# SkyworkAI/Vitron

Measured on NVIDIA H100. Metric: Vicuna-7B generated tokens/s, batch-8 x (256 vision + 512 text) prefill + 128-token greedy decode, incl. ViT-L/14 encode, higher is better.
Workload: dtype bf16

## Files before the change

### include/vitron_b200.h

```cpp
#ifndef VITRON_B200_H_
#define VITRON_B200_H_

#include <stddef.h>
#include <stdint.h>

#ifdef __cplusplus
extern "C" {
#endif

#ifndef __CUDA_RUNTIME_H__
typedef struct CUstream_st* cudaStream_t;
#endif

#define VB_ACT_NONE 0
#define VB_ACT_GELU 1
#define VB_ACT_QUICK_GELU 2
#define VB_ACT_RELU 3
#define VB_ACT_SILU 4

#define VB_GLU_NONE 0
#define VB_GLU_SWIGLU 1
#define VB_GLU_GEGLU 2

typedef struct vb_epilogue {
  const void* bias;
  const void* rowbias;
  int64_t rowbias_rows;
  const void* residual;
  int64_t ldr;
  float alpha;
  int32_t act;
  int32_t glu;
  int32_t out_fp32;
  const float* rowscale;
  float rms_eps;
} vb_epilogue;

const char* vb200_version(void);
const char* vb200_last_error(void);
int vb200_device_ok(void);
int vb200_set_pdl(int enable);
int vb200_set_attention_impl(int impl);
int vb200_attention_watchdog(uint32_t* out3);
int vb200_attention_tc_occupancy(int head_dim);

size_t vb200_gemm_bf16_workspace_size(int64_t M, int64_t N, int64_t K);
int vb200_gemm_bf16(const void* A, int64_t lda, const void* W, int64_t ldw, void* out, int64_t ldo,
                    int64_t M, int64_t N, int64_t K, const vb_epilogue* epi, void* workspace,
                    size_t workspace_bytes, cudaStream_t stream);

int vb200_gemm_nf4(const void* A, int64_t lda, const void* codes, const void* scales, const float* kscale, void* out,
                   int64_t ldo, int64_t M, int64_t N, int64_t K, const vb_epilogue* epi, cudaStream_t stream);
int vb200_nf4_dequant(const void* codes, const void* scales, const float* kscale, void* out, int64_t N, int64_t K,
                      cudaStream_t stream);



size_t vb200_conv_nhwc_workspace_size(int64_t nb, int64_t h, int64_t w, int64_t cin, int64_t cout, int kh, int kw,
                                      int stride, int pad_h, int pad_w);
int vb200_conv_nhwc_bf16(const void* X, const void* Wt, void* out, int64_t nb, int64_t h,
                         int64_t w, int64_t cin, int64_t cout, int kh, int kw, int stride,
                         int pad_h, int pad_w, const vb_epilogue* epi, void* workspace,
                         size_t workspace_bytes, cudaStream_t stream);
int vb200_set_gemm_impl(int impl);
int vb200_set_gemm_debug(int resident_b, int dbg);

int vb200_conv_nhwc_direct(const void* X, const void* Wt, const void* bias, void* out, int64_t nb,
                           int64_t h, int64_t w, int64_t cin, int64_t cout, int kh, int kw,
                           int stride, int pad_h, int pad_w, cudaStream_t stream);

int vb200_rmsnorm(const void* x, int64_t ldx, const void* weight, void* out, int64_t ldo,
                  int64_t rows, int64_t d, float eps, cudaStream_t stream);
int vb200_row_rstd(const void* x, int64_t ldx, float* out, int64_t rows, int64_t d, float eps,
                   cudaStream_t stream);
int vb200_layernorm(const void* x, int64_t ldx, const void* weight, const void* bias, void* out,
                    int64_t ldo, int64_t rows, int64_t d, float eps, cudaStream_t stream);
size_t vb200_groupnorm_workspace_size(int64_t n, int64_t groups, int64_t c);
int vb200_groupnorm_nhwc(const void* x, const void* weight, const void* bias, void* out, int64_t n,
                         int64_t spatial, int64_t c, int64_t groups, float eps, int act,
                         void* workspace, size_t workspace_bytes, cudaStream_t stream);

int vb200_attention(const void* q, const void* k, const void* v, void* out, int64_t B, int64_t H,
                    int64_t Sq, int64_t Skv, int64_t head_dim, int64_t q_sb, int64_t q_ss,
                    int64_t q_sh, int64_t k_sb, int64_t k_ss, int64_t k_sh, int64_t v_sb,
                    int64_t v_ss, int64_t v_sh, int64_t o_sb, int64_t o_ss, int64_t o_sh,
                    float scale, int causal, const int32_t* kv_len, const uint8_t* mask,
                    int64_t m_sb, int64_t m_sh, int64_t m_sq, cudaStream_t stream);
size_t vb200_attention_workspace_size(int64_t B, int64_t H, int64_t Sq, int64_t Skv, int64_t head_dim, int causal);
int vb200_attention_ws(const void* q, const void* k, const void* v, void* out, int64_t B, int64_t H,
                       int64_t Sq, int64_t Skv, int64_t head_dim, int64_t q_sb, int64_t q_ss,
                       int64_t q_sh, int64_t k_sb, int64_t k_ss, int64_t k_sh, int64_t v_sb,
                       int64_t v_ss, int64_t v_sh, int64_t o_sb, int64_t o_ss, int64_t o_sh,
                       float scale, int causal, const int32_t* kv_len, const uint8_t* mask,
                       int64_t m_sb, int64_t m_sh, int64_t m_sq, void* workspace, size_t workspace_bytes,
                       cudaStream_t stream);
size_t vb200_attention_paged_workspace_size(int64_t B, int64_t H, int64_t Sq, int64_t head_dim, int64_t max_kv_len);
int vb200_attention_paged(const void* q, int64_t q_sb, int64_t q_ss, int64_t q_sh, const void* k_pages,
                          const void* v_pages, int64_t num_pages, const int32_t* block_table, int64_t max_pages,
                          const int32_t* q_start, const int32_t* q_len, void* out, int64_t o_sb, int64_t o_ss,
                          int64_t o_sh, int64_t B, int64_t H, int64_t Sq, int64_t head_dim, int64_t page_size,
                          int64_t max_kv_len, float scale, void* workspace, size_t workspace_bytes,
                          cudaStream_t stream);
int vb200_attention_short(const void* q, const void* k, const void* v, void* out, int64_t nseq,
                          int64_t H, int64_t S, int64_t head_dim, int64_t q_sb, int64_t q_ss,
                          int64_t q_sh, int64_t k_sb, int64_t k_ss, int64_t k_sh, int64_t v_sb,
                          int64_t v_ss, int64_t v_sh, int64_t o_sb, int64_t o_ss, int64_t o_sh,
                          int64_t inner, int64_t q_so, int64_t k_so, int64_t v_so, int64_t o_so,
                          float scale, cudaStream_t stream);

int vb200_rope_kv_append(void* qkv, int64_t ld_qkv, const int32_t* positions,
                         const int32_t* batch_of_token, const int32_t* slot_of_token, void* k_pages,
                         void* v_pages, const int32_t* block_table, int64_t max_pages,
                         int64_t tokens, int64_t n_heads, int64_t head_dim, int64_t page_size,
                         float rope_theta, cudaStream_t stream);
size_t vb200_attn_decode_workspace_size(int64_t B, int64_t n_heads, int64_t head_dim,
                                        int64_t max_splits);
int vb200_attn_decode_paged(const void* q, int64_t ld_q, const void* k_pages, const void* v_pages,
                            const int32_t* block_table, int64_t max_pages, const int32_t* kv_len,
                            void* out, int64_t ld_o, int64_t B, int64_t n_heads, int64_t head_dim,
                            int64_t page_size, int64_t max_kv_len, float scale, void* workspace,
                            size_t workspace_bytes, cudaStream_t stream);
int vb200_rope_table(const int32_t* positions, float* table, int64_t B, int64_t head_dim, float rope_theta,
                     cudaStream_t stream);
int vb200_attn_decode_rope(const void* qkv, int64_t ld_qkv, const float* rope_table, void* k_pages,
                           void* v_pages, const int32_t* block_table, int64_t max_pages,
                           const int32_t* kv_len, void* out, int64_t ld_o, int64_t B, int64_t n_heads,
                           int64_t head_dim, int64_t page_size, int64_t max_kv_len, float scale,
                           void* workspace, size_t workspace_bytes, cudaStream_t stream);
int vb200_attn_decode_rope_beam(const void* qkv, int64_t ld_qkv, const float* rope_table, void* k_pages,
                                void* v_pages, const int32_t* block_table, int64_t max_pages, const int32_t* kv_len,
                                const int32_t* beam_src, int64_t src_ld, const int32_t* gen_start, void* out,
                                int64_t ld_o, int64_t B, int64_t n_heads, int64_t head_dim, int64_t page_size,
// ... 101 lines not shown
```

### vitron_b200/_lib.py

```python
import ctypes as C
import os

_HERE = os.path.dirname(os.path.abspath(__file__))
LIB_PATH = os.path.join(_HERE, "libvitron_b200.so")

ACT_NONE, ACT_GELU, ACT_QUICK_GELU, ACT_RELU, ACT_SILU = 0, 1, 2, 3, 4
GLU_NONE, GLU_SWIGLU, GLU_GEGLU = 0, 1, 2

_ERR = {-1: "VB_ERR_ARG", -2: "VB_ERR_CUDA", -3: "VB_ERR_WORKSPACE", -4: "VB_ERR_UNSUPPORTED",
        -5: "VB_ERR_DRIVER"}


class Epilogue(C.Structure):
    _fields_ = [
        ("bias", C.c_void_p), ("rowbias", C.c_void_p), ("rowbias_rows", C.c_int64),
        ("residual", C.c_void_p), ("ldr", C.c_int64), ("alpha", C.c_float),
        ("act", C.c_int32), ("glu", C.c_int32), ("out_fp32", C.c_int32),
        ("rowscale", C.c_void_p), ("rms_eps", C.c_float),
    ]


_p, _i64, _i32, _f, _sz = C.c_void_p, C.c_int64, C.c_int, C.c_float, C.c_size_t

SIGNATURES = {
    "vb200_version": (C.c_char_p, []),
    "vb200_last_error": (C.c_char_p, []),
    "vb200_device_ok": (_i32, []),
    "vb200_set_pdl": (_i32, [_i32]),
    "vb200_set_attention_impl": (_i32, [_i32]),
    "vb200_attention_watchdog": (_i32, [_p]),
    "vb200_attention_tc_occupancy": (_i32, [_i32]),
    "vb200_gemm_bf16_workspace_size": (_sz, [_i64, _i64, _i64]),
    "vb200_gemm_bf16": (_i32, [_p, _i64, _p, _i64, _p, _i64, _i64, _i64, _i64, C.POINTER(Epilogue), _p, _sz, _p]),
    "vb200_gemm_nf4": (_i32, [_p, _i64, _p, _p, _p, _p, _i64, _i64, _i64, _i64, C.POINTER(Epilogue), _p]),
    "vb200_nf4_dequant": (_i32, [_p, _p, _p, _p, _i64, _i64, _p]),
    "vb200_conv_nhwc_workspace_size": (_sz, [_i64, _i64, _i64, _i64, _i64, _i32, _i32, _i32, _i32, _i32]),
    "vb200_conv_nhwc_bf16": (_i32, [_p, _p, _p, _i64, _i64, _i64, _i64, _i64, _i32, _i32, _i32, _i32, _i32,
                                    C.POINTER(Epilogue), _p, _sz, _p]),
    "vb200_set_gemm_impl": (_i32, [_i32]),
    "vb200_set_gemm_debug": (_i32, [_i32, _i32]),
    "vb200_conv_nhwc_direct": (_i32, [_p, _p, _p, _p, _i64, _i64, _i64, _i64, _i64, _i32, _i32, _i32, _i32, _i32, _p]),
    "vb200_rmsnorm": (_i32, [_p, _i64, _p, _p, _i64, _i64, _i64, _f, _p]),
    "vb200_row_rstd": (_i32, [_p, _i64, _p, _i64, _i64, _f, _p]),
    "vb200_layernorm": (_i32, [_p, _i64, _p, _p, _p, _i64, _i64, _i64, _f, _p]),
    "vb200_groupnorm_workspace_size": (_sz, [_i64, _i64, _i64]),
    "vb200_groupnorm_nhwc": (_i32, [_p, _p, _p, _p, _i64, _i64, _i64, _i64, _f, _i32, _p, _sz, _p]),
    "vb200_attention": (_i32, [_p, _p, _p, _p, _i64, _i64, _i64, _i64, _i64] + [_i64] * 12 +
                        [_f, _i32, _p, _p, _i64, _i64, _i64, _p]),
    "vb200_attention_workspace_size": (_sz, [_i64, _i64, _i64, _i64, _i64, _i32]),
    "vb200_attention_ws": (_i32, [_p, _p, _p, _p, _i64, _i64, _i64, _i64, _i64] + [_i64] * 12 +
                           [_f, _i32, _p, _p, _i64, _i64, _i64, _p, _sz, _p]),
    "vb200_attention_paged_workspace_size": (_sz, [_i64, _i64, _i64, _i64, _i64]),
    "vb200_attention_paged": (_i32, [_p, _i64, _i64, _i64, _p, _p, _i64, _p, _i64, _p, _p, _p, _i64, _i64, _i64,
                                     _i64, _i64, _i64, _i64, _i64, _i64, _f, _p, _sz, _p]),
    "vb200_attention_short": (_i32, [_p, _p, _p, _p, _i64, _i64, _i64, _i64] + [_i64] * 17 + [_f, _p]),
    "vb200_add_rowgroup": (_i32, [_p, _p, _p, _i64, _i64, _i64, _i64, _p]),
    "vb200_rope_kv_append": (_i32, [_p, _i64, _p, _p, _p, _p, _p, _p, _i64, _i64, _i64, _i64, _i64, _f, _p]),
    "vb200_attn_decode_workspace_size": (_sz, [_i64, _i64, _i64, _i64]),
    "vb200_attn_decode_paged": (_i32, [_p, _i64, _p, _p, _p, _i64, _p, _p, _i64, _i64, _i64, _i64, _i64, _i64,
                                       _f, _p, _sz, _p]),
    "vb200_rope_table": (_i32, [_p, _p, _i64, _i64, _f, _p]),
    "vb200_attn_decode_rope": (_i32, [_p, _i64, _p, _p, _p, _p, _i64, _p, _p, _i64, _i64, _i64, _i64, _i64, _i64,
                                      _f, _p, _sz, _p]),
    "vb200_attn_decode_rope_beam": (_i32, [_p, _i64, _p, _p, _p, _p, _i64, _p, _p, _i64, _p, _p, _i64, _i64, _i64, _i64,
                                           _i64, _i64, _f, _p, _sz, _p]),
    "vb200_splice_multimodal": (_i32, [_p, _i64, _p, _i64, _p, _p, _i64, _i64, _p]),
    "vb200_argmax_rows": (_i32, [_p, _i32, _i64, _i64, _i64, _p, _p]),
    "vb200_argmax_advance": (_i32, [_p, _i64, _i64, _i64, _p, _p, _p, _p, _p, _i64, _p, _p]),
    "vb200_sample_advance": (_i32, [_p, _i64, _i64, _i64, _p, _p, _p, _p, _p, _p, _i64, _p, _p]),
    "vb200_beam_workspace_size": (_sz, [_i64]),
    "vb200_beam_advance": (_i32, [_p, _i64, _i64, _i64, _i64, _p, _p, _p, _p, _p, _i64, _p, _p, _p, _p, _p, _i64, _p, _p,
                                  _p, _p, _i64, _p, _p, _sz, _p]),
    "vb200_beam_sample_advance": (_i32, [_p, _i64, _i64, _i64, _i64, _p, _p, _p, _p, _p, _i64, _p, _p, _p, _p, _p, _i64,
                                         _p, _p, _p, _p, _i64, _p, _p, _sz, _p, _p]),
    "vb200_patchify": (_i32, [_p, _i32, _p, _i64, _i64, _i64, _i64, _i64, _i64, _p]),
    "vb200_vit_embed_ln": (_i32, [_p, _p, _p, _p, _p, _p, _i64, _i64, _i64, _f, _p]),
    "vb200_upsample2x_nhwc": (_i32, [_p, _p, _i64, _i64, _i64, _i64, _p]),
    "vb200_add_bf16": (_i32, [_p, _p, _p, _i64, _i64, _p]),
    "vb200_cfg_combine": (_i32, [_p, _p, _p, _f, _i64, _p]),
    "vb200_region_mask_pool": (_i32, [_p, _p, _p, _i64, _i64, _i64, _i64, _p]),
    "vb200_seem_attn_mask": (_i32, [_p, _p, _i64, _i64, _i64, _i64, _i64, _p]),
    "vb200_resize_bilinear_nhwc": (_i32, [_p, _p, _i64, _i64, _i64, _i64, _i64, _i64, _p]),
    "vb200_softmax_rows": (_i32, [_p, _i64, _p, _i64, _i64, _i64, _p]),
    "vb200_preprocess_frames": (_i32, [_p, _p] + [_i64] * 11 + [_p, _p, _i32, _i32, _i32, _p]),
    "vb200_im2col_nchw": (_i32, [_p, _i32, _p] + [_i64] * 10 + [_p]),
    "vb200_set_dwconv_impl": (_i32, [_i32]),
    "vb200_dwconv_nhwc": (_i32, [_p, _i64, _p, _p, _i64, _i64, _i64, _i64, _i64, _i32, _p]),
    "vb200_colmean_workspace_size": (_sz, [_i64, _i64, _i64]),
    "vb200_colmean": (_i32, [_p, _p, _i64, _i64, _i64, _i32, _p, _sz, _p]),
    "vb200_focal_modulate": (_i32, [_p, _i64, _p, _i64, _p, _p, _i64, _i64, _i64, _f, _p]),
    "vb200_mul_rows": (_i32, [_p, _i64, _p, _i64, _p, _i64, _i64, _p]),
    "vb200_layernorm_add": (_i32, [_p, _i64, _p, _p, _p, _i64, _p, _i64, _i64, _i64, _f, _p]),
}

_lib = None


def load():
    global _lib
    if _lib is not None:
        return _lib
    if not os.path.exists(LIB_PATH):
        raise RuntimeError(
            f"{LIB_PATH} is missing: build it with `python -m vitron_b200.build` "
            "(nvcc, sm_90a). vitron_b200 has no CPU fallback.")
    lib = C.CDLL(LIB_PATH)
    for name, (res, args) in SIGNATURES.items():
        fn = getattr(lib, name)
        fn.restype = res
        fn.argtypes = args
    _lib = lib
    mode = os.environ.get("VB200_GEMM_MODE")
    if mode:
# ... 13 lines not shown
```

### vitron_b200/csrc/gemm.cu

```cuda
#include <cstdlib>
#include "gemm_v2.cuh"

namespace vb {

__global__ void splitk_reduce_kernel(const float* __restrict__ ws, int splits,
                                     long long split_stride, long long ws_ld, int rows, int ncols,
                                     void* out, long long ldo, const bf16* __restrict__ bias,
                                     const bf16* __restrict__ rowbias, int rowbias_rows,
                                     const bf16* __restrict__ residual, long long ldr, float alpha,
                                     int act, int glu, int out_fp32, const float* __restrict__ rowscale) {
  pdl_trigger();
  pdl_wait();
  const int n_out_total = glu != VB_GLU_NONE ? ncols / 2 : ncols;
  const int groups = (n_out_total + 7) / 8;
  long long idx = blockIdx.x * static_cast<long long>(blockDim.x) + threadIdx.x;
  if (idx >= static_cast<long long>(rows) * groups) return;
  reduce_item(ws, splits, split_stride, ws_ld, static_cast<int>(idx / groups), static_cast<int>(idx % groups) * 8,
              ncols, out, ldo, bias, rowbias, rowbias_rows, residual, ldr, alpha, act, glu, out_fp32, rowscale);
}

typedef CUresult (*PFN_encodeTiled)(CUtensorMap*, CUtensorMapDataType, cuuint32_t, void*,
                                    const cuuint64_t*, const cuuint64_t*, const cuuint32_t*,
                                    const cuuint32_t*, CUtensorMapInterleave, CUtensorMapSwizzle,
                                    CUtensorMapL2promotion, CUtensorMapFloatOOBfill);

static PFN_encodeTiled get_encode_fn() {
  static PFN_encodeTiled fn = nullptr;
  if (fn) return fn;
  void* p = nullptr;
  cudaDriverEntryPointQueryResult q;
  if (cudaGetDriverEntryPoint("cuTensorMapEncodeTiled", &p, cudaEnableDefault, &q) != cudaSuccess ||
      q != cudaDriverEntryPointSuccess)
    return nullptr;
  fn = reinterpret_cast<PFN_encodeTiled>(p);
  return fn;
}

static int make_tmap(CUtensorMap* m, const void* ptr, int rank, const uint64_t* dims,
                     const uint64_t* strides_bytes , const uint32_t* box,
                     const uint32_t* estr, CUtensorMapSwizzle swz = CU_TENSOR_MAP_SWIZZLE_128B) {
  PFN_encodeTiled fn = get_encode_fn();
  if (!fn) return VB_ERR_DRIVER;
  CUresult r = fn(m, CU_TENSOR_MAP_DATA_TYPE_BFLOAT16, rank, const_cast<void*>(ptr), dims,
                  strides_bytes, box, estr, CU_TENSOR_MAP_INTERLEAVE_NONE, swz,
                  CU_TENSOR_MAP_L2_PROMOTION_L2_256B, CU_TENSOR_MAP_FLOAT_OOB_FILL_NONE);
  return r == CUDA_SUCCESS ? VB_OK : VB_ERR_DRIVER;
}


static int swap_splits(long long M, long long N, long long K) {
  const int sms = vb_num_sms();
  const int m_blocks = static_cast<int>((N + BLOCK_M - 1) / BLOCK_M);
  const int kblocks = static_cast<int>((K + BLOCK_K - 1) / BLOCK_K);
  int best = 1;
  float best_score = -1.f;
  for (int s = 1; s <= 32 && s <= kblocks; ++s) {
    if (static_cast<size_t>(s) * M * N * sizeof(float) > (static_cast<size_t>(96) << 20)) break;
    const long long units = static_cast<long long>(m_blocks) * s;
    const long long waves = (units + sms - 1) / sms;
    const float util = static_cast<float>(units) / static_cast<float>(waves * sms);
    const int per = (kblocks + s - 1) / s;
    const float bal = static_cast<float>(kblocks) / static_cast<float>(s * per);
    const float score = util * bal - 0.01f * static_cast<float>(s);
    if (score > best_score + 1e-6f) { best_score = score; best = s; }
  }
  return best;
}

static int validate_epi(const vb_epilogue* e, long long N) {
  if (e->glu != VB_GLU_NONE && (N % 32) != 0) return VB_ERR_ARG;
  if (e->act < VB_ACT_NONE || e->act > VB_ACT_SILU) return VB_ERR_ARG;
  if (e->glu < VB_GLU_NONE || e->glu > VB_GLU_GEGLU) return VB_ERR_ARG;
  return VB_OK;
}

static int g_gemm_impl = 0;
static int g_gemm_resb = 1;
static int g_gemm_dbg = 0;
int resb_smem_bytes(int bn, int nkb);

static int resb_tile(long long M, long long N, int nkb, int need) {
  if (g_gemm_impl == 1 || !(g_gemm_resb & 3) || (need != 0 && need != F_RES && need != F_GLU && need != F_ACT)) return 0;
  if (nkb > 5 && !(g_gemm_resb & 2)) return 0;
  if (M < 4096) return 0;
  const int cands[3] = {160, 256, 128};
  int best = 0;
  float best_cost = 1e30f;
  for (int i = 0; i < 3; ++i) {
    const int bn = cands[i];
    if (resb_smem_bytes(bn, nkb) > SMEM_LIMIT) continue;
    const long long nb = (N + bn - 1) / bn;
    if (nb > vb_num_sms()) continue;
    const int groups = vb_num_sms() / static_cast<int>(nb);
    const long long mb = (M + BLOCK_M - 1) / BLOCK_M;
    const long long per_cta = (mb + groups - 1) / groups;
    const float mma = static_cast<float>(bn) / 256.f, astream = bn == 160 ? 0.55f : 0.9f;
    const float cost = static_cast<float>(per_cta) * nkb * (mma > astream ? mma : astream);
    if (cost < best_cost) { best_cost = cost; best = bn; }
  }
  return best;
}

struct TilePlan {
  int bn, splits;
};

static TilePlan plan_tiles(long long mb, long long N, int kblocks, bool allow_split, long long out_rows) {
  const int sms = vb_num_sms();
  const int cands[5] = {256, 160, 128, 64, 32};
  const float tk[5] = {1.0f, 0.78f, 0.76f, 0.625f, 0.57f};
  TilePlan best = {256, 1};
  float best_t = 1e30f;
  if (const char* force = getenv("VB200_FORCE_BN")) {
    const int v = atoi(force);
    if (v == 256 || v == 160 || v == 128 || v == 64 || v == 32) return {v, 1};
  }
  for (int i = 0; i < 5; ++i) {
    const int bn = cands[i];
    const long long nbk = (N + bn - 1) / bn;
    const long long tiles = mb * nbk;
    for (int sp = 1; sp <= 8; ++sp) {
// ... 285 lines not shown
```

### vitron_b200/csrc/gemv.cu

```cuda
#include "common.cuh"
#include "vitron_b200.h"
#include <type_traits>

namespace vb {

struct GemvParams {
  const bf16* W; long long ldw;
  const bf16* X; long long ldx;
  void* out; long long ldo;
  int M, N, K;
  const bf16* bias; const bf16* rowbias; int rowbias_rows;
  const bf16* residual; long long ldr;
  float alpha; int act, glu, out_fp32;
  const float* rowscale; float rms_eps;
};

__device__ __forceinline__ float gemv_act(float x, int act) {
  switch (act) {
    case VB_ACT_GELU: return gelu_erf(x);
    case VB_ACT_QUICK_GELU: return quick_gelu(x);
    case VB_ACT_RELU: return fmaxf(x, 0.f);
    case VB_ACT_SILU: return silu(x);
    default: return x;
  }
}

__device__ __forceinline__ void mma16816(float (&c)[4], uint32_t a0, uint32_t a1, uint32_t a2, uint32_t a3,
                                         uint32_t b0, uint32_t b1) {
  asm("mma.sync.aligned.m16n8k16.row.col.f32.bf16.bf16.f32 {%0,%1,%2,%3}, {%4,%5,%6,%7}, {%8,%9}, {%0,%1,%2,%3};"
      : "+f"(c[0]), "+f"(c[1]), "+f"(c[2]), "+f"(c[3])
      : "r"(a0), "r"(a1), "r"(a2), "r"(a3), "r"(b0), "r"(b1));
}

__device__ __forceinline__ uint4 ldg_stream(const bf16* p, bool ok) {
  uint4 v = make_uint4(0, 0, 0, 0);
  if (ok) asm volatile("ld.global.nc.L1::no_allocate.v4.u32 {%0,%1,%2,%3}, [%4];" : "=r"(v.x), "=r"(v.y), "=r"(v.z), "=r"(v.w) : "l"(p));
  return v;
}
__device__ __forceinline__ uint4 ldg_cached(const bf16* p, bool ok) {
  uint4 v = make_uint4(0, 0, 0, 0);
  if (ok) v = __ldg(reinterpret_cast<const uint4*>(p));
  return v;
}

template <int ROWS, int NT>
__global__ void __launch_bounds__(256, 2) gemv_bf16_kernel(const GemvParams p) {
  constexpr int WARPS = 8;
  constexpr int RG = ROWS / 16;
  constexpr int KS = WARPS / RG;
  constexpr int G = 2;
  __shared__ float red[2][WARPS][16][NT * 8 + 1];
  __shared__ float red_sq[WARPS][NT * 8];
  __shared__ float rstd_s[NT * 8];

  const int warp = threadIdx.x >> 5, lane = threadIdx.x & 31;
  const int g = lane >> 2, t = lane & 3;
  const int rg = warp % RG, ks = warp / RG;
  const int ntiles = (p.N + ROWS - 1) / ROWS;
  const bf16* x0 = p.X + static_cast<long long>(min(g, p.M - 1)) * p.ldx;
  const bf16* x1 = p.X + static_cast<long long>(min(g + 8, p.M - 1)) * p.ldx;
  const bool x0ok = g < p.M, x1ok = (NT == 2) && (g + 8 < p.M);

  const int chunks = (p.K + 63) / 64;
  const int base = chunks / KS, rem = chunks % KS;
  const int c0 = ks * base + min(ks, rem);
  const int c1 = c0 + base + (ks < rem ? 1 : 0);
  const int ngroups = (c1 - c0 + G - 1) / G;
  const int npairs = (ngroups + 1) / 2;

  const bool do_rms = p.rms_eps > 0.f && p.rowscale == nullptr;
  float sq0 = 0.f, sq1 = 0.f;

  struct Buf { uint4 wl[G][2], wh[G][2]; };
  auto load_group = [&](Buf& bf, int tile, int grp) {
    const int row0 = tile * ROWS + rg * 16;
    const bf16* wa = p.W + static_cast<long long>(min(row0 + g, p.N - 1)) * p.ldw;
    const bf16* wb = p.W + static_cast<long long>(min(row0 + g + 8, p.N - 1)) * p.ldw;
    const bool live = tile < ntiles;
#pragma unroll
    for (int u = 0; u < G; ++u) {
      const int c = c0 + grp * G + u;
      const int k0 = c * 64 + 8 * t, k1 = k0 + 32;
      const bool in = live && c < c1;
      const bool ok0 = in && k0 < p.K, ok1 = in && k1 < p.K;
      bf.wl[u][0] = ldg_stream(wa + k0, ok0); bf.wl[u][1] = ldg_stream(wa + k1, ok1);
      bf.wh[u][0] = ldg_stream(wb + k0, ok0); bf.wh[u][1] = ldg_stream(wb + k1, ok1);
    }
  };
  float acc[NT][4];
  auto compute_group = [&](const Buf& bf, int grp, bool first_tile) {
    uint4 xa[G][2], xb[G][2];
#pragma unroll
    for (int u = 0; u < G; ++u) {
      const int c = c0 + grp * G + u;
      const int k0 = c * 64 + 8 * t, k1 = k0 + 32;
      const bool in = c < c1;
      const bool ok0 = in && k0 < p.K, ok1 = in && k1 < p.K;
      xa[u][0] = ldg_cached(x0 + k0, ok0 && x0ok); xa[u][1] = ldg_cached(x0 + k1, ok1 && x0ok);
      if (NT == 2) { xb[u][0] = ldg_cached(x1 + k0, ok0 && x1ok); xb[u][1] = ldg_cached(x1 + k1, ok1 && x1ok); }
    }
#pragma unroll
    for (int u = 0; u < G; ++u) {
      const uint32_t al[8] = {bf.wl[u][0].x, bf.wl[u][0].y, bf.wl[u][0].z, bf.wl[u][0].w, bf.wl[u][1].x, bf.wl[u][1].y, bf.wl[u][1].z, bf.wl[u][1].w};
      const uint32_t ah[8] = {bf.wh[u][0].x, bf.wh[u][0].y, bf.wh[u][0].z, bf.wh[u][0].w, bf.wh[u][1].x, bf.wh[u][1].y, bf.wh[u][1].z, bf.wh[u][1].w};
      const uint32_t b0[8] = {xa[u][0].x, xa[u][0].y, xa[u][0].z, xa[u][0].w, xa[u][1].x, xa[u][1].y, xa[u][1].z, xa[u][1].w};
      uint32_t b1[8] = {0, 0, 0, 0, 0, 0, 0, 0};
      if (NT == 2) {
        b1[0] = xb[u][0].x; b1[1] = xb[u][0].y; b1[2] = xb[u][0].z; b1[3] = xb[u][0].w;
        b1[4] = xb[u][1].x; b1[5] = xb[u][1].y; b1[6] = xb[u][1].z; b1[7] = xb[u][1].w;
      }
      if (do_rms && first_tile && rg == 0) {
#pragma unroll
        for (int j = 0; j < 8; ++j) {
          float2 f = unpack_bf16(b0[j]);
          sq0 += f.x * f.x + f.y * f.y;
          if (NT == 2) { float2 h2 = unpack_bf16(b1[j]); sq1 += h2.x * h2.x + h2.y * h2.y; }
        }
      }
#pragma unroll
      for (int j = 0; j < 4; ++j) {
        mma16816(acc[0], al[2 * j], ah[2 * j], al[2 * j + 1], ah[2 * j + 1], b0[2 * j], b0[2 * j + 1]);
        if (NT == 2) mma16816(acc[1], al[2 * j], ah[2 * j], al[2 * j + 1], ah[2 * j + 1], b1[2 * j], b1[2 * j + 1]);
      }
    }
  };

  Buf buf0, buf1;
  pdl_trigger();
  load_group(buf0, blockIdx.x, 0);
  load_group(buf1, blockIdx.x, 1);
  pdl_wait();

  const bool glu = p.glu != VB_GLU_NONE;
  const int out_cols = glu ? ROWS / 2 : ROWS;
  const int n_out_total = glu ? p.N / 2 : p.N;
  int par = 0;
  bool first = true;
  for (int tile = blockIdx.x; tile < ntiles; tile += gridDim.x) {
#pragma unroll
    for (int i = 0; i < NT; ++i) acc[i][0] = acc[i][1] = acc[i][2] = acc[i][3] = 0.f;
    for (int pr = 0; pr < npairs; ++pr) {
      const bool last = pr + 1 == npairs;
      compute_group(buf0, 2 * pr, first);
      if (!last) load_group(buf0, tile, 2 * pr + 2); else load_group(buf0, tile + gridDim.x, 0);
      compute_group(buf1, 2 * pr + 1, first);
      if (!last) load_group(buf1, tile, 2 * pr + 3); else load_group(buf1, tile + gridDim.x, 1);
    }
#pragma unroll
    for (int i = 0; i < NT; ++i) {
      red[par][warp][g][i * 8 + 2 * t] = acc[i][0];
      red[par][warp][g][i * 8 + 2 * t + 1] = acc[i][1];
      red[par][warp][g + 8][i * 8 + 2 * t] = acc[i][2];
      red[par][warp][g + 8][i * 8 + 2 * t + 1] = acc[i][3];
    }
    if (do_rms && first) {
      sq0 += __shfl_xor_sync(0xffffffffu, sq0, 1); sq0 += __shfl_xor_sync(0xffffffffu, sq0, 2);
      if (NT == 2) { sq1 += __shfl_xor_sync(0xffffffffu, sq1, 1); sq1 += __shfl_xor_sync(0xffffffffu, sq1, 2); }
      if (t == 0) { red_sq[warp][g] = sq0; if (NT == 2) red_sq[warp][8 + g] = sq1; }
    }
    __syncthreads();
    if (do_rms && first) {
      if (threadIdx.x < NT * 8) {
        float ss = 0.f;
#pragma unroll
        for (int s2 = 0; s2 < KS; ++s2) ss += red_sq[s2 * RG][threadIdx.x];
        rstd_s[threadIdx.x] = rsqrtf(ss / p.K + p.rms_eps);
      }
      __syncthreads();
    }
    for (int item = threadIdx.x; item < p.M * out_cols; item += 256) {
      const int tok = item / out_cols, j = item % out_cols;
      const int fa = j, fb = j + 16;
      const int na = tile * ROWS + fa;
      const int oc = glu ? tile * (ROWS / 2) + j : na;
      if (oc >= n_out_total) continue;
      float va = 0.f, vb_ = 0.f;
#pragma unroll
      for (int s2 = 0; s2 < KS; ++s2) {
        va += red[par][s2 * RG + fa / 16][fa % 16][tok];
        if (glu) vb_ += red[par][s2 * RG + (fb / 16) % RG][fb % 16][tok];
      }
      if (do_rms) { const float rs = rstd_s[tok]; va *= rs; vb_ *= rs; }
      else if (p.rowscale) { const float rs = p.rowscale[tok]; va *= rs; vb_ *= rs; }
      if (p.bias) {
        va += __bfloat162float(p.bias[na]);
        if (glu) vb_ += __bfloat162float(p.bias[na + 16]);
      }
      if (p.rowbias) {
        const bf16* rbp = p.rowbias + (tok / p.rowbias_rows) * static_cast<long long>(p.N);
        va += __bfloat162float(rbp[na]);
        if (glu) vb_ += __bfloat162float(rbp[na + 16]);
      }
      float r;
      if (p.glu == VB_GLU_SWIGLU) r = silu(va) * vb_;
      else if (p.glu == VB_GLU_GEGLU) r = va * gelu_erf(vb_);
      else r = gemv_act(va, p.act);
      if (p.residual) r = __bfloat162float(p.residual[tok * p.ldr + oc]) + p.alpha * r;
      else r *= p.alpha;
      if (p.out_fp32) reinterpret_cast<float*>(p.out)[tok * p.ldo + oc] = r;
      else reinterpret_cast<bf16*>(p.out)[tok * p.ldo + oc] = __float2bfloat16(r);
    }
    par ^= 1;
    first = false;
  }
}

}

using namespace vb;

int vb_launch_gemv(const void* A, int64_t lda, const void* W, int64_t ldw, void* out, int64_t ldo, int64_t M,
                   int64_t N, int64_t K, const vb_epilogue* e, cudaStream_t stream) {
  GemvParams p;
  p.W = reinterpret_cast<const bf16*>(W); p.ldw = ldw;
  p.X = reinterpret_cast<const bf16*>(A); p.ldx = lda;
  p.out = out; p.ldo = ldo;
  p.M = static_cast<int>(M); p.N = static_cast<int>(N); p.K = static_cast<int>(K);
  p.bias = reinterpret_cast<const bf16*>(e->bias);
  p.rowbias = reinterpret_cast<const bf16*>(e->rowbias);
  p.rowbias_rows = e->rowbias_rows > 0 ? static_cast<int>(e->rowbias_rows) : 1;
  p.residual = reinterpret_cast<const bf16*>(e->residual); p.ldr = e->ldr;
  p.alpha = e->alpha; p.act = e->act; p.glu = e->glu; p.out_fp32 = e->out_fp32;
  p.rowscale = e->rowscale; p.rms_eps = e->rms_eps;
  const bool glu = e->glu != VB_GLU_NONE;
  const bool rows32 = glu || (N / 16 > 6LL * vb_num_sms());
  const unsigned tiles = static_cast<unsigned>((N + (rows32 ? 31 : 15)) / (rows32 ? 32 : 16));
  const unsigned cap = 2u * static_cast<unsigned>(vb_num_sms());
  const unsigned grid = tiles < cap ? tiles : cap;
  cudaError_t err;
  if (M <= 8) {
    if (rows32) err = vb_launch(gemv_bf16_kernel<32, 1>, dim3(grid), dim3(256), 0, stream, p);
    else err = vb_launch(gemv_bf16_kernel<16, 1>, dim3(grid), dim3(256), 0, stream, p);
  } else {
    if (rows32) err = vb_launch(gemv_bf16_kernel<32, 2>, dim3(grid), dim3(256), 0, stream, p);
    else err = vb_launch(gemv_bf16_kernel<16, 2>, dim3(grid), dim3(256), 0, stream, p);
  }
  if (err != cudaSuccess) { vb_set_last_error(err); return VB_ERR_CUDA; }
  return VB_OK;
}
```

### vitron_b200/ops.py

```python
import ctypes as C
import math
import struct

import torch

from . import _lib, beam
from .nf4 import NF4Weight
from ._lib import (ACT_GELU, ACT_NONE, ACT_QUICK_GELU, ACT_RELU, ACT_SILU, GLU_GEGLU, GLU_NONE,
                   GLU_SWIGLU, Epilogue, check)

BF16 = torch.bfloat16
_ws = {}
_launches = [0]


def launch_count():
    return _launches[0]


def count_launches(n):
    _launches[0] += int(n)


def _stream():
# ... 259 lines not shown
    check(lib.vb200_layernorm(x2.data_ptr(), ldx, weight.data_ptr(), _ptr(bias), o2.data_ptr(), ldo, x2.shape[0],
                              x2.shape[1], float(eps), _stream()), "vb200_layernorm")
    _launches[0] += 1
    return out


def groupnorm_nhwc(x, weight, bias, groups, eps, act=ACT_NONE, n=None, out=None):
    lib = _lib.load()
    _req(x.is_contiguous() and x.dtype == BF16, "x must be contiguous bf16")
    c = x.shape[-1]
    n = x.shape[0] if n is None else n
    spatial = x.numel() // (n * c)
    out = torch.empty_like(x) if out is None else out
    need = lib.vb200_groupnorm_workspace_size(n, groups, c)
    ws = workspace(need, x.device, "gn")
    check(lib.vb200_groupnorm_nhwc(x.data_ptr(), weight.data_ptr(), bias.data_ptr(), out.data_ptr(), n, spatial, c,
                                   groups, float(eps), int(act), ws.data_ptr(), need, _stream()),
          "vb200_groupnorm_nhwc")
    _launches[0] += 1
    return out


def _bsh(t):
    _req(t.dim() == 4 and t.stride(3) == 1, "expect [B, S, H, D] with contiguous D")
    return t.stride(0), t.stride(1), t.stride(2)


def attention(q, k, v, scale=None, causal=False, kv_len=None, mask=None, out=None):
    lib = _lib.load()
    B, Sq, H, D = q.shape
    Skv = k.shape[1]
    scale = 1.0 / math.sqrt(D) if scale is None else scale
    if out is None:
        out = torch.empty((B, Sq, H, D), dtype=BF16, device=q.device)
    m_ptr, m_sb, m_sh, m_sq = 0, 0, 0, 0
    if mask is not None:
        if mask.dtype == torch.bool:
            mask = mask.view(torch.uint8)
        _req(mask.dim() == 4 and mask.stride(3) == 1 and mask.shape[2] == Sq and mask.shape[3] == Skv, "bad mask")
        m_ptr = mask.data_ptr()
        m_sb = mask.stride(0) if mask.shape[0] > 1 else 0
        m_sh = mask.stride(1) if mask.shape[1] > 1 else 0
        m_sq = mask.stride(2)
    need = lib.vb200_attention_workspace_size(B, H, Sq, Skv, D, 1 if causal else 0) if kv_len is None else 0
    ws = workspace(need, q.device, "attn") if need else None
    check(lib.vb200_attention_ws(q.data_ptr(), k.data_ptr(), v.data_ptr(), out.data_ptr(), B, H, Sq, Skv, D,
                                 *_bsh(q), *_bsh(k), *_bsh(v), *_bsh(out), float(scale), 1 if causal else 0,
                                 _ptr(kv_len), m_ptr, m_sb, m_sh, m_sq, _ptr(ws), need, _stream()), "vb200_attention_ws")
    _launches[0] += 2 if need else 1
    return out


def attention_paged(q, k_pages, v_pages, block_table, q_start, q_len, max_kv_len, scale=None, out=None):
    lib = _lib.load()
    B, Sq, H, D = q.shape
    scale = 1.0 / math.sqrt(D) if scale is None else scale
    _req(block_table.dim() == 2 and block_table.shape[0] >= B and block_table.is_contiguous(),
         "block_table: contiguous int32 [>= B, max_pages]")
    _req(k_pages.is_contiguous() and v_pages.is_contiguous() and k_pages.shape == v_pages.shape, "contiguous pages")
    if out is None:
        out = torch.empty((B, Sq, H, D), dtype=BF16, device=q.device)
    need = lib.vb200_attention_paged_workspace_size(B, H, Sq, D, int(max_kv_len))
    ws = workspace(need, q.device, "attn") if need else None
    check(lib.vb200_attention_paged(q.data_ptr(), *_bsh(q), k_pages.data_ptr(), v_pages.data_ptr(), k_pages.shape[0],
                                    block_table.data_ptr(), block_table.shape[1], q_start.data_ptr(), q_len.data_ptr(),
                                    out.data_ptr(), *_bsh(out), B, H, Sq, D, k_pages.shape[2], int(max_kv_len),
                                    float(scale), _ptr(ws), need, _stream()), "vb200_attention_paged")
    _launches[0] += 2 if need else 1
    return out


def set_attention_impl(impl):
    check(_lib.load().vb200_set_attention_impl(int(impl)), "vb200_set_attention_impl")


def attention_watchdog():
    import ctypes
    buf = (ctypes.c_uint32 * 3)()
    torch.cuda.synchronize()
    check(_lib.load().vb200_attention_watchdog(ctypes.addressof(buf)), "vb200_attention_watchdog")
    return tuple(buf)


def attention_short(q, k, v, scale=None, out=None):
    lib = _lib.load()
    scale = 1.0 / math.sqrt(q.shape[-1]) if scale is None else scale
    if out is None:
        out = torch.empty(q.shape, dtype=BF16, device=q.device)
    if q.dim() == 4:
        nseq, S, H, D = q.shape
        inner, so = 0, (0, 0, 0, 0)
        b3 = [_bsh(t) for t in (q, k, v, out)]
    else:
        _req(q.dim() == 5, "expect 4-D or 5-D q")
        outer, inner, S, H, D = q.shape
        nseq = outer * inner
        so = tuple(t.stride(0) for t in (q, k, v, out))
        for t in (q, k, v, out):
            _req(t.stride(4) == 1, "contiguous head dim")
        b3 = [(t.stride(1), t.stride(2), t.stride(3)) for t in (q, k, v, out)]
    check(lib.vb200_attention_short(q.data_ptr(), k.data_ptr(), v.data_ptr(), out.data_ptr(), nseq, H, S, D,
                                    *b3[0], *b3[1], *b3[2], *b3[3], inner, *so, float(scale), _stream()),
          "vb200_attention_short")
    _launches[0] += 1
    return out


def add_rowgroup(x, table, group_rows, period, out=None):
    lib = _lib.load()
    x2, _ = _rows2d(x)
    _req(x.is_contiguous() and table.is_contiguous(), "contiguous")
    out = torch.empty_like(x) if out is None else out
    check(lib.vb200_add_rowgroup(x2.data_ptr(), table.data_ptr(), out.data_ptr(), x2.shape[0], x2.shape[1],
                                 group_rows, period, _stream()), "vb200_add_rowgroup")
    _launches[0] += 1
    return out


def rope_kv_append(qkv, positions, n_heads, head_dim, theta, k_pages=None, v_pages=None, block_table=None,
                   batch_of_token=None, slot_of_token=None, page_size=0):
    lib = _lib.load()
    q2, ld = _rows2d(qkv)
    max_pages = block_table.shape[1] if block_table is not None else 0
    check(lib.vb200_rope_kv_append(q2.data_ptr(), ld, positions.data_ptr(), _ptr(batch_of_token),
                                   _ptr(slot_of_token), _ptr(k_pages), _ptr(v_pages), _ptr(block_table),
                                   max_pages, q2.shape[0], n_heads, head_dim, page_size, float(theta), _stream()),
          "vb200_rope_kv_append")
    _launches[0] += 1
    return qkv


def attn_decode_paged(q, k_pages, v_pages, block_table, kv_len, n_heads, head_dim, page_size, max_kv_len,
                      scale=None, out=None):
    lib = _lib.load()
    B = q.shape[0]
    scale = 1.0 / math.sqrt(head_dim) if scale is None else scale
    if out is None:
        out = torch.empty((B, n_heads * head_dim), dtype=BF16, device=q.device)
    need = lib.vb200_attn_decode_workspace_size(B, n_heads, head_dim, 32)
    ws = workspace(need, q.device, "dec")
    check(lib.vb200_attn_decode_paged(q.data_ptr(), q.stride(0), k_pages.data_ptr(), v_pages.data_ptr(),
                                      block_table.data_ptr(), block_table.shape[1], kv_len.data_ptr(),
                                      out.data_ptr(), out.stride(0), B, n_heads, head_dim, page_size, max_kv_len,
                                      float(scale), ws.data_ptr(), need, _stream()), "vb200_attn_decode_paged")
    _launches[0] += 1
    return out


def rope_table(positions, head_dim, theta, out=None):
    lib = _lib.load()
    B = positions.shape[0]
    if out is None:
        out = torch.empty((B, head_dim), dtype=torch.float32, device=positions.device)
    check(lib.vb200_rope_table(positions.data_ptr(), out.data_ptr(), B, head_dim, float(theta), _stream()),
          "vb200_rope_table")
    _launches[0] += 1
    return out


def attn_decode_rope(qkv, table, k_pages, v_pages, block_table, kv_len, n_heads, head_dim, page_size, max_kv_len,
                     scale=None, out=None):
    lib = _lib.load()
    B = qkv.shape[0]
    scale = 1.0 / math.sqrt(head_dim) if scale is None else scale
    if out is None:
        out = torch.empty((B, n_heads * head_dim), dtype=BF16, device=qkv.device)
# ... 361 lines not shown
```

Before: 1030.

## Stream GEMV weights through per-warp TMA mbarrier ring instead of register double-buffering

Replaces the register-level double-buffered streaming loads of weight tiles in the decode GEMV kernel with a per-warp 4-stage TMA ring in swizzled shared memory, synchronised by mbarriers. Weight prefetch for the first stages is issued before the PDL wait so it overlaps the previous kernel. The aim is deeper memory-level parallelism with fewer registers spent on in-flight loads. It adds about 66KB of dynamic shared memory per block, which may limit occupancy to fewer blocks per SM, a tensor-map encode on every launch, and a watchdog trap path plus occupancy query helpers.

```diff
diff --git a/include/vitron_b200.h b/include/vitron_b200.h
--- a/include/vitron_b200.h
+++ b/include/vitron_b200.h
@@ -48,6 +48,8 @@
 int vb200_gemm_bf16(const void* A, int64_t lda, const void* W, int64_t ldw, void* out, int64_t ldo,
                     int64_t M, int64_t N, int64_t K, const vb_epilogue* epi, void* workspace,
                     size_t workspace_bytes, cudaStream_t stream);
+int vb200_gemv_watchdog(uint32_t* out3);
+int vb200_gemv_occupancy(int32_t m, int32_t rows32);
 
 int vb200_gemm_nf4(const void* A, int64_t lda, const void* codes, const void* scales, const float* kscale, void* out,
                    int64_t ldo, int64_t M, int64_t N, int64_t K, const vb_epilogue* epi, cudaStream_t stream);
diff --git a/vitron_b200/_lib.py b/vitron_b200/_lib.py
--- a/vitron_b200/_lib.py
+++ b/vitron_b200/_lib.py
@@ -29,6 +29,8 @@
     "vb200_set_pdl": (_i32, [_i32]),
     "vb200_set_attention_impl": (_i32, [_i32]),
     "vb200_attention_watchdog": (_i32, [_p]),
+    "vb200_gemv_watchdog": (_i32, [_p]),
+    "vb200_gemv_occupancy": (_i32, [_i32, _i32]),
     "vb200_attention_tc_occupancy": (_i32, [_i32]),
     "vb200_gemm_bf16_workspace_size": (_sz, [_i64, _i64, _i64]),
     "vb200_gemm_bf16": (_i32, [_p, _i64, _p, _i64, _p, _i64, _i64, _i64, _i64, C.POINTER(Epilogue), _p, _sz, _p]),
diff --git a/vitron_b200/csrc/gemm.cu b/vitron_b200/csrc/gemm.cu
--- a/vitron_b200/csrc/gemm.cu
+++ b/vitron_b200/csrc/gemm.cu
@@ -36,7 +36,7 @@
   return fn;
 }
 
-static int make_tmap(CUtensorMap* m, const void* ptr, int rank, const uint64_t* dims,
+int make_tmap(CUtensorMap* m, const void* ptr, int rank, const uint64_t* dims,
                      const uint64_t* strides_bytes , const uint32_t* box,
                      const uint32_t* estr, CUtensorMapSwizzle swz = CU_TENSOR_MAP_SWIZZLE_128B) {
   PFN_encodeTiled fn = get_encode_fn();
diff --git a/vitron_b200/csrc/gemv.cu b/vitron_b200/csrc/gemv.cu
--- a/vitron_b200/csrc/gemv.cu
+++ b/vitron_b200/csrc/gemv.cu
@@ -5,7 +5,6 @@
 namespace vb {
 
 struct GemvParams {
-  const bf16* W; long long ldw;
   const bf16* X; long long ldx;
   void* out; long long ldo;
   int M, N, K;
@@ -32,34 +31,59 @@
       : "r"(a0), "r"(a1), "r"(a2), "r"(a3), "r"(b0), "r"(b1));
 }
 
-__device__ __forceinline__ uint4 ldg_stream(const bf16* p, bool ok) {
-  uint4 v = make_uint4(0, 0, 0, 0);
-  if (ok) asm volatile("ld.global.nc.L1::no_allocate.v4.u32 {%0,%1,%2,%3}, [%4];" : "=r"(v.x), "=r"(v.y), "=r"(v.z), "=r"(v.w) : "l"(p));
-  return v;
-}
 __device__ __forceinline__ uint4 ldg_cached(const bf16* p, bool ok) {
   uint4 v = make_uint4(0, 0, 0, 0);
   if (ok) v = __ldg(reinterpret_cast<const uint4*>(p));
   return v;
 }
+__device__ __forceinline__ uint4 lds128(uint32_t addr) {
+  uint4 v;
+  asm volatile("ld.shared.v4.u32 {%0,%1,%2,%3}, [%4];" : "=r"(v.x), "=r"(v.y), "=r"(v.z), "=r"(v.w) : "r"(addr));
+  return v;
+}
+
+__device__ unsigned int g_gemv_watchdog[4];
+
+__device__ __noinline__ void gemv_wait_slow(uint64_t* bar, uint32_t parity) {
+  unsigned long long t0, t;
+  asm volatile("mov.u64 %0, %%globaltimer;" : "=l"(t0));
+  while (!mbar_try_wait(bar, parity)) {
+    asm volatile("mov.u64 %0, %%globaltimer;" : "=l"(t));
+    if (t - t0 > 4000000000ull) {
+      if (atomicCAS(&g_gemv_watchdog[0], 0u, 1u) == 0u) {
+        g_gemv_watchdog[1] = blockIdx.x;
+        g_gemv_watchdog[2] = threadIdx.x;
+      }
+      __threadfence_system();
+      __trap();
+    }
+  }
+}
+__device__ __forceinline__ void gemv_wait(uint64_t* bar, uint32_t parity) {
+  if (!mbar_try_wait(bar, parity)) gemv_wait_slow(bar, parity);
+}
+
+constexpr int GEMV_STAGES = 4;
+constexpr int GEMV_STAGE_BYTES = 16 * 64 * 2;
+constexpr int GEMV_RING_BYTES = 8 * GEMV_STAGES * GEMV_STAGE_BYTES;
+constexpr int GEMV_SMEM_BYTES = GEMV_RING_BYTES + 8 * GEMV_STAGES * 8 + 1024;
 
 template <int ROWS, int NT>
-__global__ void __launch_bounds__(256, 2) gemv_bf16_kernel(const GemvParams p) {
+__global__ void __launch_bounds__(256, 2) gemv_bf16_kernel(const __grid_constant__ CUtensorMap wmap, const GemvParams p) {
   constexpr int WARPS = 8;
   constexpr int RG = ROWS / 16;
   constexpr int KS = WARPS / RG;
   constexpr int G = 2;
+  constexpr int STAGES = GEMV_STAGES;
   __shared__ float red[2][WARPS][16][NT * 8 + 1];
   __shared__ float red_sq[WARPS][NT * 8];
   __shared__ float rstd_s[NT * 8];
+  extern __shared__ uint8_t gemv_smem_raw[];
 
   const int warp = threadIdx.x >> 5, lane = threadIdx.x & 31;
   const int g = lane >> 2, t = lane & 3;
   const int rg = warp % RG, ks = warp / RG;
   const int ntiles = (p.N + ROWS - 1) / ROWS;
-  const bf16* x0 = p.X + static_cast<long long>(min(g, p.M - 1)) * p.ldx;
-  const bf16* x1 = p.X + static_cast<long long>(min(g + 8, p.M - 1)) * p.ldx;
-  const bool x0ok = g < p.M, x1ok = (NT == 2) && (g + 8 < p.M);
 
   const int chunks = (p.K + 63) / 64;
   const int base = chunks / KS, rem = chunks % KS;
@@ -68,41 +92,65 @@
   const int ngroups = (c1 - c0 + G - 1) / G;
   const int npairs = (ngroups + 1) / 2;
 
+  uint8_t* smem = reinterpret_cast<uint8_t*>((reinterpret_cast<uintptr_t>(gemv_smem_raw) + 1023) & ~uintptr_t(1023));
+  const uint32_t ring = smem_u32(smem) + warp * STAGES * GEMV_STAGE_BYTES;
+  uint64_t* full = reinterpret_cast<uint64_t*>(smem + GEMV_RING_BYTES) + warp * STAGES;
+  const int nchunks = c1 - c0;
+  const int my_tiles = (ntiles - 1 - static_cast<int>(blockIdx.x)) / static_cast<int>(gridDim.x) + 1;
+  const int total = my_tiles * nchunks;
+  auto issue = [&](int seq) {
+    const int tl = seq / nchunks;
+    const int c = c0 + (seq - tl * nchunks);
+    const int tile = static_cast<int>(blockIdx.x) + tl * static_cast<int>(gridDim.x);
+    const int st = seq % STAGES;
+    mbar_arrive_expect_tx(full + st, GEMV_STAGE_BYTES);
+    tma_load_2d(smem + (warp * STAGES + st) * GEMV_STAGE_BYTES, &wmap, full + st, c * 64, tile * ROWS + rg * 16);
+  };
+
+  pdl_trigger();
+  if (lane == 0) {
+    prefetch_tmap(&wmap);
+    for (int st = 0; st < STAGES; ++st) mbar_init(full + st, 1);
+    fence_barrier_init();
+    for (int seq = 0; seq < STAGES && seq < total; ++seq) issue(seq);
+  }
+  __syncwarp();
+  pdl_wait();
+
+  const bf16* x0 = p.X + static_cast<long long>(min(g, p.M - 1)) * p.ldx;
+  const bf16* x1 = p.X + static_cast<long long>(min(g + 8, p.M - 1)) * p.ldx;
+  const bool x0ok = g < p.M, x1ok = (NT == 2) && (g + 8 < p.M);
   const bool do_rms = p.rms_eps > 0.f && p.rowscale == nullptr;
   float sq0 = 0.f, sq1 = 0.f;
-
-  struct Buf { uint4 wl[G][2], wh[G][2]; };
-  auto load_group = [&](Buf& bf, int tile, int grp) {
-    const int row0 = tile * ROWS + rg * 16;
-    const bf16* wa = p.W + static_cast<long long>(min(row0 + g, p.N - 1)) * p.ldw;
-    const bf16* wb = p.W + static_cast<long long>(min(row0 + g + 8, p.N - 1)) * p.ldw;
-    const bool live = tile < ntiles;
-#pragma unroll
-    for (int u = 0; u < G; ++u) {
-      const int c = c0 + grp * G + u;
-      const int k0 = c * 64 + 8 * t, k1 = k0 + 32;
-      const bool in = live && c < c1;
-      const bool ok0 = in && k0 < p.K, ok1 = in && k1 < p.K;
-      bf.wl[u][0] = ldg_stream(wa + k0, ok0); bf.wl[u][1] = ldg_stream(wa + k1, ok1);
-      bf.wh[u][0] = ldg_stream(wb + k0, ok0); bf.wh[u][1] = ldg_stream(wb + k1, ok1);
-    }
-  };
+  const uint32_t frag_lo = g * 128 + ((t ^ (g & 7)) << 4), frag_lo2 = g * 128 + (((t + 4) ^ (g & 7)) << 4);
+  const uint32_t frag_hi = frag_lo + 8 * 128, frag_hi2 = frag_lo2 + 8 * 128;
+  int seq = 0;
+
   float acc[NT][4];
-  auto compute_group = [&](const Buf& bf, int grp, bool first_tile) {
-    uint4 xa[G][2], xb[G][2];
+  auto compute_group = [&](int grp, bool first_tile) {
+    uint4 wl[G][2], wh[G][2], xa[G][2], xb[G][2];
 #pragma unroll
     for (int u = 0; u < G; ++u) {
       const int c = c0 + grp * G + u;
       const int k0 = c * 64 + 8 * t, k1 = k0 + 32;
       const bool in = c < c1;
       const bool ok0 = in && k0 < p.K, ok1 = in && k1 < p.K;
+      if (in) {
+        const int st = (seq + u) % STAGES;
+        gemv_wait(full + st, ((seq + u) / STAGES) & 1);
+        const uint32_t sb = ring + st * GEMV_STAGE_BYTES;
+        wl[u][0] = lds128(sb + frag_lo); wl[u][1] = lds128(sb + frag_lo2);
+        wh[u][0] = lds128(sb + frag_hi); wh[u][1] = lds128(sb + frag_hi2);
+      } else {
+        wl[u][0] = wl[u][1] = wh[u][0] = wh[u][1] = make_uint4(0, 0, 0, 0);
+      }
       xa[u][0] = ldg_cached(x0 + k0, ok0 && x0ok); xa[u][1] = ldg_cached(x0 + k1, ok1 && x0ok);
       if (NT == 2) { xb[u][0] = ldg_cached(x1 + k0, ok0 && x1ok); xb[u][1] = ldg_cached(x1 + k1, ok1 && x1ok); }
     }
 #pragma unroll
     for (int u = 0; u < G; ++u) {
-      const uint32_t al[8] = {bf.wl[u][0].x, bf.wl[u][0].y, bf.wl[u][0].z, bf.wl[u][0].w, bf.wl[u][1].x, bf.wl[u][1].y, bf.wl[u][1].z, bf.wl[u][1].w};
-      const uint32_t ah[8] = {bf.wh[u][0].x, bf.wh[u][0].y, bf.wh[u][0].z, bf.wh[u][0].w, bf.wh[u][1].x, bf.wh[u][1].y, bf.wh[u][1].z, bf.wh[u][1].w};
+      const uint32_t al[8] = {wl[u][0].x, wl[u][0].y, wl[u][0].z, wl[u][0].w, wl[u][1].x, wl[u][1].y, wl[u][1].z, wl[u][1].w};
+      const uint32_t ah[8] = {wh[u][0].x, wh[u][0].y, wh[u][0].z, wh[u][0].w, wh[u][1].x, wh[u][1].y, wh[u][1].z, wh[u][1].w};
       const uint32_t b0[8] = {xa[u][0].x, xa[u][0].y, xa[u][0].z, xa[u][0].w, xa[u][1].x, xa[u][1].y, xa[u][1].z, xa[u][1].w};
       uint32_t b1[8] = {0, 0, 0, 0, 0, 0, 0, 0};
       if (NT == 2) {
@@ -123,13 +171,15 @@
         if (NT == 2) mma16816(acc[1], al[2 * j], ah[2 * j], al[2 * j + 1], ah[2 * j + 1], b1[2 * j], b1[2 * j + 1]);
       }
     }
+    const int used = min(G, max(0, c1 - (c0 + grp * G)));
+    __syncwarp();
+    if (lane == 0 && used > 0) {
+      fence_proxy_async_smem();
+      for (int u = 0; u < used; ++u)
+        if (seq + u + STAGES < total) issue(seq + u + STAGES);
+    }
+    seq += used;
   };
-
-  Buf buf0, buf1;
-  pdl_trigger();
-  load_group(buf0, blockIdx.x, 0);
-  load_group(buf1, blockIdx.x, 1);
-  pdl_wait();
 
   const bool glu = p.glu != VB_GLU_NONE;
   const int out_cols = glu ? ROWS / 2 : ROWS;
@@ -140,11 +190,8 @@
 #pragma unroll
     for (int i = 0; i < NT; ++i) acc[i][0] = acc[i][1] = acc[i][2] = acc[i][3] = 0.f;
     for (int pr = 0; pr < npairs; ++pr) {
-      const bool last = pr + 1 == npairs;
-      compute_group(buf0, 2 * pr, first);
-      if (!last) load_group(buf0, tile, 2 * pr + 2); else load_group(buf0, tile + gridDim.x, 0);
-      compute_group(buf1, 2 * pr + 1, first);
-      if (!last) load_group(buf1, tile, 2 * pr + 3); else load_group(buf1, tile + gridDim.x, 1);
+      compute_group(2 * pr, first);
+      compute_group(2 * pr + 1, first);
     }
 #pragma unroll
     for (int i = 0; i < NT; ++i) {
@@ -207,12 +254,29 @@
 
 }
 
+namespace vb {
+int make_tmap(CUtensorMap* m, const void* ptr, int rank, const uint64_t* dims, const uint64_t* strides_bytes,
+              const uint32_t* box, const uint32_t* estr, CUtensorMapSwizzle swz);
+}
+
 using namespace vb;
+
+template <int ROWS, int NT>
+static cudaError_t set_gemv_smem() {
+  static cudaError_t e = cudaFuncSetAttribute(gemv_bf16_kernel<ROWS, NT>, cudaFuncAttributeMaxDynamicSharedMemorySize,
+                                              GEMV_SMEM_BYTES);
+  return e;
+}
+
+template <int ROWS, int NT>
+static cudaError_t launch_gemv(const CUtensorMap& wmap, const GemvParams& p, unsigned grid, cudaStream_t stream) {
+  if (cudaError_t e = set_gemv_smem<ROWS, NT>()) return e;
+  return vb_launch(gemv_bf16_kernel<ROWS, NT>, dim3(grid), dim3(256), GEMV_SMEM_BYTES, stream, wmap, p);
+}
 
 int vb_launch_gemv(const void* A, int64_t lda, const void* W, int64_t ldw, void* out, int64_t ldo, int64_t M,
                    int64_t N, int64_t K, const vb_epilogue* e, cudaStream_t stream) {
   GemvParams p;
-  p.W = reinterpret_cast<const bf16*>(W); p.ldw = ldw;
   p.X = reinterpret_cast<const bf16*>(A); p.ldx = lda;
   p.out = out; p.ldo = ldo;
   p.M = static_cast<int>(M); p.N = static_cast<int>(N); p.K = static_cast<int>(K);
@@ -222,19 +286,48 @@
   p.residual = reinterpret_cast<const bf16*>(e->residual); p.ldr = e->ldr;
   p.alpha = e->alpha; p.act = e->act; p.glu = e->glu; p.out_fp32 = e->out_fp32;
   p.rowscale = e->rowscale; p.rms_eps = e->rms_eps;
+  CUtensorMap wmap;
+  const uint64_t dims[2] = {static_cast<uint64_t>((K + 7) / 8 * 8), static_cast<uint64_t>(N)};
+  const uint64_t strides[1] = {static_cast<uint64_t>(ldw) * 2};
+  const uint32_t box[2] = {64, 16}, estr[2] = {1, 1};
+  if (int r = make_tmap(&wmap, W, 2, dims, strides, box, estr, CU_TENSOR_MAP_SWIZZLE_128B)) return r;
   const bool glu = e->glu != VB_GLU_NONE;
   const bool rows32 = glu || (N / 16 > 6LL * vb_num_sms());
   const unsigned tiles = static_cast<unsigned>((N + (rows32 ? 31 : 15)) / (rows32 ? 32 : 16));
   const unsigned cap = 2u * static_cast<unsigned>(vb_num_sms());
   const unsigned grid = tiles < cap ? tiles : cap;
   cudaError_t err;
-  if (M <= 8) {
-    if (rows32) err = vb_launch(gemv_bf16_kernel<32, 1>, dim3(grid), dim3(256), 0, stream, p);
-    else err = vb_launch(gemv_bf16_kernel<16, 1>, dim3(grid), dim3(256), 0, stream, p);
-  } else {
-    if (rows32) err = vb_launch(gemv_bf16_kernel<32, 2>, dim3(grid), dim3(256), 0, stream, p);
-    else err = vb_launch(gemv_bf16_kernel<16, 2>, dim3(grid), dim3(256), 0, stream, p);
-  }
+  if (M <= 8) err = rows32 ? launch_gemv<32, 1>(wmap, p, grid, stream) : launch_gemv<16, 1>(wmap, p, grid, stream);
+  else err = rows32 ? launch_gemv<32, 2>(wmap, p, grid, stream) : launch_gemv<16, 2>(wmap, p, grid, stream);
   if (err != cudaSuccess) { vb_set_last_error(err); return VB_ERR_CUDA; }
   return VB_OK;
 }
+
+extern "C" int vb200_gemv_watchdog(uint32_t* out3) {
+  VB_CHECK_ARG(out3);
+  unsigned int h[4] = {0, 0, 0, 0};
+  cudaError_t e = cudaMemcpyFromSymbol(h, g_gemv_watchdog, sizeof(h));
+  if (e != cudaSuccess) { vb_set_last_error(e); return VB_ERR_CUDA; }
+  out3[0] = h[0]; out3[1] = h[1]; out3[2] = h[2];
+  if (h[0]) {
+    unsigned int z[4] = {0, 0, 0, 0};
+    cudaMemcpyToSymbol(g_gemv_watchdog, z, sizeof(z));
+  }
+  return VB_OK;
+}
+
+template <int ROWS, int NT>
+static int gemv_occupancy() {
+  int n = 0;
+  cudaError_t e = set_gemv_smem<ROWS, NT>();
+  if (e == cudaSuccess)
+    e = cudaOccupancyMaxActiveBlocksPerMultiprocessor(&n, gemv_bf16_kernel<ROWS, NT>, 256, GEMV_SMEM_BYTES);
+  if (e != cudaSuccess) { vb_set_last_error(e); return VB_ERR_CUDA; }
+  return n;
+}
+
+extern "C" int vb200_gemv_occupancy(int32_t m, int32_t rows32) {
+  if (m < 1 || m > 16) return VB_ERR_ARG;
+  if (m <= 8) return rows32 ? gemv_occupancy<32, 1>() : gemv_occupancy<16, 1>();
+  return rows32 ? gemv_occupancy<32, 2>() : gemv_occupancy<16, 2>();
+}
diff --git a/vitron_b200/ops.py b/vitron_b200/ops.py
--- a/vitron_b200/ops.py
+++ b/vitron_b200/ops.py
@@ -365,6 +365,21 @@
     return tuple(buf)
 
 
+def gemv_watchdog():
+    import ctypes
+    buf = (ctypes.c_uint32 * 3)()
+    torch.cuda.synchronize()
+    check(_lib.load().vb200_gemv_watchdog(ctypes.addressof(buf)), "vb200_gemv_watchdog")
+    return tuple(buf)
+
+
+def gemv_occupancy(m, rows32):
+    r = _lib.load().vb200_gemv_occupancy(int(m), 1 if rows32 else 0)
+    if r < 0:
+        check(r, "vb200_gemv_occupancy")
+    return r
+
+
 def attention_short(q, k, v, scale=None, out=None):
     lib = _lib.load()
     scale = 1.0 / math.sqrt(q.shape[-1]) if scale is None else scale
```

New measurement: 1037, median of 6. No clear change (+0.7%).
